# RunpeiDong/ACT

Measured on AMD Instinct MI355X. Metric: stage2_pretrain_point_clouds_per_sec, higher is better.
Workload: dtype f32

## Files before the change

act_amd/_abi.py:

```python
import ctypes

_vp, _i, _f, _sz = ctypes.c_void_p, ctypes.c_int, ctypes.c_float, ctypes.c_size_t
_u, _u64, _ll, _str = ctypes.c_uint, ctypes.c_uint64, ctypes.c_longlong, ctypes.c_char_p
_d = ctypes.c_double
_P = ctypes.POINTER


class GemmEpilogue(ctypes.Structure):
    _fields_ = [("alpha", _f), ("act", _i), ("accumulate", _i), ("rows_per_scale", _i), ("ldr", _i), ("ldaux", _i),
                ("res_row_div", _i), ("bias", _vp), ("rowscale", _vp), ("res", _vp), ("aux", _vp)]


class GemmTnProblem(ctypes.Structure):
    _fields_ = [("A", _vp), ("lda", _i), ("B", _vp), ("ldb", _i), ("C", _vp), ("ldc", _i), ("M", _i), ("N", _i), ("bias_out", _vp)]


class GemmFx(ctypes.Structure):
    _fields_ = ([(n, _vp) for n in ("a_scale", "a_shift", "b_scale", "b_shift", "tile_stats", "gmax", "garg")] + [("group", _i), ("store_c", _i)]
                + [(n, _vp) for n in ("sa_src", "sa_arg", "ep_src", "ep_arg", "row_groups")])


class BlockParams(ctypes.Structure):
    _fields_ = [(n, _vp) for n in ("norm1_w", "norm1_b", "qkv_w", "qkv_b", "proj_w", "proj_b", "norm2_w", "norm2_b",
                                   "fc1_w", "fc1_b", "fc2_w", "fc2_b")]
# ... 129 lines not shown
    "act_group_max_bwd_wgrad_workspace": (_sz, [_i, _i, _i, _i]),
    "act_group_max_bwd_wgrad_f32": [_vp, _vp, _i, _i, _i, _vp, _i, _i, _vp, _vp, _vp, _i, _vp, _sz, _vp],
    "act_group_sum_f32": [_vp, _i, _i, _i, _vp, _vp],
    "act_edge_gn_lrelu_max_f32": [_vp, _i, _i, _vp, _i, _i, _i, _i, _i, _vp, _vp, _f, _f, _vp, _vp, _i, _i, _vp],
    "act_edge_gn_lrelu_max_bwd_f32": [_vp, _i, _i, _vp, _i, _i, _i, _i, _i, _vp, _vp, _vp, _f, _vp, _i, _vp, _vp, _vp, _vp],
    "act_edge_bwd_lds": [_i],
    "act_gn_gumbel_argmax_gather_f32": [_vp, _i, _i, _i, _i, _vp, _vp, _f, _f, _vp, _u64, _vp, _f, _vp, _i, _vp, _vp, _vp, _vp, _vp],
    "act_gumbel_softmax_fwd_f32": [_vp, _i, _i, _vp, _u64, _f, _vp, _vp],
    "act_gumbel_softmax_bwd_f32": [_vp, _vp, _i, _i, _f, _vp, _vp],
    "act_kl_uniform_fwd_f32": [_vp, _i, _i, _i, _vp, _vp, _vp, _vp],
    "act_kl_uniform_bwd_f32": [_vp, _vp, _vp, _vp, _i, _i, _i, _vp, _vp],
    "act_split_bf16x2_f32": [_vp, _i, _i, _i, _vp, _vp, _vp],
    "act_sgemm_nt_bf16x3_supported": [_i, _i, _i],
    "act_sgemm_nt_bf16x3_f32": [_i, _i, _i, _vp, _vp, _vp, _vp, _vp, _i, _epi, _vp],
    "act_layernorm_fwd_planes_f32": [_vp, _vp, _vp, _vp, _vp, _vp, _vp, _vp, _vp, _vp, _i, _i, _f, _vp],
    "act_prompt_layernorm_fwd_planes_f32": [_vp, _vp, _i, _i, _i, _f, _u64, _vp, _vp, _vp, _f, _vp, _vp, _vp],
    "act_attention_fwd_prefix_planes_f32": [_vp, _i, _vp, _i, _vp, _vp, _vp, _vp, _i, _i, _i, _f, _vp],
    "act_sgemm_nt_bf16x3_planes_f32": [_i, _i, _i, _vp, _vp, _vp, _vp, _vp, _i, _vp, _vp, _epi, _vp],
    "act_split_f16x2_f32": [_vp, _i, _i, _i, _f, _vp, _vp, _vp, _vp],
    "act_sgemm_nt_f16x3_supported": [_i, _i, _i],
    "act_sgemm_nt_f16x3_planes_f32": [_i, _i, _i, _vp, _vp, _f, _vp, _vp, _vp, _vp, _i, _vp, _vp, _f, _epi, _vp],
    "act_sgemm_nt_f16x3_pick_tile": [_i, _i, _i, _i],
    "act_sgemm_nt_f16x3_planes_tile_f32": [_i, _i, _i, _vp, _vp, _f, _vp, _vp, _vp, _vp, _i, _vp, _vp, _f, _epi, _vp, _i],
    "act_layernorm_fwd_f16_planes_f32": [_vp, _vp, _vp, _vp, _vp, _vp, _vp, _vp, _f, _vp, _vp, _i, _i, _f, _vp],
    "act_attention_fwd_prefix_f16_planes_f32": [_vp, _i, _vp, _i, _vp, _vp, _vp, _f, _vp, _i, _i, _i, _f, _vp],
    "act_split_f16x2_affine_relu_f32": [_vp, _i, _i, _i, _vp, _vp, _f, _vp, _vp, _vp],
    "act_sgemm_nt_f16x3_gmax_supported": [_i, _i, _i, _i],
    "act_sgemm_nt_f16x3_gmax_pick_tile": [_i, _i, _i, _i],
    "act_sgemm_nt_f16x3_gmax_f32": [_i, _i, _i, _vp, _i, _vp, _vp, _vp, _vp, _f, _vp, _vp, _vp, _vp, _i, _vp, _i, _i, _vp],
    "act_gemm_tune_set": [_i] * 7,
    "act_gemm_tune_get": [_i] * 5 + [_P(_i), _P(_i)],
    "act_gemm_tune_clear": [],
    "act_gemm_tile_info": [_i] + [_P(_i)] * 4,
    "act_scale_rows_f32": [_vp, _vp, _i, _i, _i, _vp, _vp],
    "act_bn_eval_affine_f32": [_vp, _vp, _vp, _vp, _f, _i, _vp, _vp, _vp],
    "act_composite_collect_begin": [],
    "act_composite_collect_end": [_P(_i), _i],
    "act_composite_shutdown": [],
    "act_block_saved_floats": (_sz, [_dims]),
    "act_block_fwd_f32": [_dims, _blk, _vp, _vp, _vp, _vp, _i, _vp, _vp, _vp, _sz, _vp],
    "act_block_bwd_scratch_floats": (_sz, [_dims]),
    "act_block_bwd_f32": [_dims, _blk, _vp, _vp, _vp, _vp, _vp, _blk, _vp, _vp, _sz, _vp, _sz, _vp, _vp],
    "act_block_stack_saved_floats": (_sz, [_dims, _i, _i]),
    "act_block_stack_bwd_scratch_floats": (_sz, [_dims, _i]),
    "act_block_stack_fwd_f32": [_dims, _P(BlockStack), _vp, _vp, _i, _vp, _vp, _vp, _sz, _vp],
    "act_block_stack_bwd_f32": [_dims, _P(BlockStack), _vp, _vp, _vp, _vp, _vp, _vp, _vp, _vp, _sz, _vp, _sz, _vp, _vp],
# ... 108 lines not shown
```

act_amd/csrc/gemm_bf16x3.hip:

```cpp
#include "gemm_common.h"
#include "split_planes.h"
#include <stdlib.h>

typedef short bf16x8 __attribute__((ext_vector_type(8)));
typedef _Float16 f16x8 __attribute__((ext_vector_type(8)));
typedef unsigned u32x4v __attribute__((ext_vector_type(4)));

namespace {

__device__ __forceinline__ float4 x3_affine_relu4(const float4& a, const float4& sc, const float4& sh) {
    return make_float4(fmaxf(__builtin_fmaf(a.x, sc.x, sh.x), 0.f), fmaxf(__builtin_fmaf(a.y, sc.y, sh.y), 0.f),
                       fmaxf(__builtin_fmaf(a.z, sc.z, sh.z), 0.f), fmaxf(__builtin_fmaf(a.w, sc.w, sh.w), 0.f));
}
__device__ __forceinline__ float4 x3_scale4(const float4& a, float s) { return make_float4(a.x * s, a.y * s, a.z * s, a.w * s); }

template <bool F16, bool AFF = false>
__global__ __launch_bounds__(256) void split_planes_kernel(const float* __restrict__ x, int K4, int ldx, long long n4, float scale,
                                                           const float* __restrict__ row_scale, unsigned short* __restrict__ p1, unsigned short* __restrict__ p2,
                                                           const float* __restrict__ col_scale = nullptr, const float* __restrict__ col_shift = nullptr) {
    for (long long i = (long long)blockIdx.x * blockDim.x + threadIdx.x; i < n4; i += (long long)gridDim.x * blockDim.x) {
        const long long row = i / K4; const int c4 = (int)(i - row * K4);
        const float4 v = *reinterpret_cast<const float4*>(x + row * ldx + c4 * 4);
        if constexpr (AFF) {
            const float4 sc = x3_scale4(*reinterpret_cast<const float4*>(col_scale + c4 * 4), scale), sh = x3_scale4(*reinterpret_cast<const float4*>(col_shift + c4 * 4), scale);
// ... 21 lines not shown
__device__ __forceinline__ void x3_affine_split8(const u32x4v& a0, const u32x4v& a1, const float* sc, const float* sh, u32x4v& h1, u32x4v& h2) {
#pragma unroll
    for (int half = 0; half < 2; ++half) {
        const float4 c = *reinterpret_cast<const float4*>(sc + half * (LROW / 2)), s = *reinterpret_cast<const float4*>(sh + half * (LROW / 2));
        const float4 v = x3_affine_relu4(__builtin_bit_cast(float4, half ? a1 : a0), c, s);
        const float e[4] = {v.x, v.y, v.z, v.w};
        unsigned h[4], l[4];
#pragma unroll
        for (int j = 0; j < 4; ++j) split_f16x2(e[j], h[j], l[j]);
        h1[2 * half] = h[0] | (h[1] << 16); h1[2 * half + 1] = h[2] | (h[3] << 16);
        h2[2 * half] = l[0] | (l[1] << 16); h2[2 * half + 1] = l[2] | (l[3] << 16);
        __builtin_amdgcn_sched_barrier(0);
    }
}

template <bool F16>
__device__ __forceinline__ f32x4 x3_mfma(const bf16x8& b, const bf16x8& a, const f32x4& c) {
    if constexpr (F16) return __builtin_amdgcn_mfma_f32_16x16x32_f16(__builtin_bit_cast(f16x8, b), __builtin_bit_cast(f16x8, a), c, 0, 0, 0);
    else return __builtin_amdgcn_mfma_f32_16x16x32_bf16(b, a, c, 0, 0, 0);
}

constexpr int x3_wgs_per_cu(int waves) { return waves <= 4 ? 2 : 1; }

template <int BM, int BN, int WGM, int WGN, int ACT, bool PLANES, bool F16, bool A32 = false, bool GMAX = false>
__global__ __launch_bounds__(64 * WGM * WGN, x3_wgs_per_cu(WGM * WGN) * WGM * WGN / 4) void sgemm_nt_bf16x3_kernel(const X3Params p) {
    static_assert(F16 || !(A32 || GMAX), "the on-load split and the group max belong to the f16 form");
    static_assert(!GMAX || (BM / WGM == 64 && !PLANES), "a group of 32 or 64 rows lies inside one wave's 64-row block");
    constexpr int NT = 64 * WGM * WGN, RP = NT / 4;
    constexpr int WM = BM / WGM, WN = BN / WGN;
    constexpr int TM = WM / 16, TN = WN / 16;
    constexpr int PA = BM * LROW, PB = BN * LROW;
    constexpr int NA = (BM + RP - 1) / RP, NB = (BN + RP - 1) / RP;
    constexpr int STAGE = 2 * (PA + PB);
    static_assert(WM % 16 == 0 && WN % 16 == 0 && BM % 16 == 0 && BN % 16 == 0, "whole 16 x 16 blocks per wave, whole waves per staging row test");
    __shared__ __attribute__((aligned(16))) unsigned short L[2 * STAGE];
    const int tid = threadIdx.x, lane = tid & 63, wave = tid >> 6;
    const int wm = wave / WGN, wn = wave % WGN;
    const int tiles_n = p.N / BN, tiles_m = p.M / BM;
    int wg = blockIdx.x;
    {
        const int nwg = tiles_m * tiles_n, q = nwg >> 3, r = nwg & 7, xcd = wg & 7, loc = wg >> 3;
        wg = (xcd < r ? xcd * (q + 1) : r * (q + 1) + (xcd - r) * q) + loc;
    }
    constexpr int GM = 8;
    const int per_group = GM * tiles_n, group = wg / per_group, first_m = group * GM;
    const int gsz = min(tiles_m - first_m, GM), in_group = wg - group * per_group;
    const int tile_m = first_m + in_group % gsz, tile_n = in_group / gsz;
    const int m0 = tile_m * BM, n0 = tile_n * BN;
    const int K = p.K, ntiles = K / BK, last = ntiles - 1;

    constexpr int X = F16 ? 1 : 0;
    f32x4 acc[X + 1][TM][TN];
#pragma unroll
    for (int x = 0; x <= X; ++x)
// ... 25 lines not shown
                RA[s_][i_] = *reinterpret_cast<const u32x4v*>(gA[s_] + (X3_WHOLE(i_, BM) ? (long long)(RP * i_) * K : ta) + (T) * BK);  \
        _Pragma("unroll") for (int i_ = 0; i_ < NB; ++i_)                                                                              \
            RB[s_][i_] = *reinterpret_cast<const u32x4v*>(gB[s_] + (X3_WHOLE(i_, BN) ? (long long)(RP * i_) * K : tb) + (T) * BK);      \
    }
#define X3_STORE(RA, RB, STG, T)                                                                                                       \
    if constexpr (A32) {                                                                                                               \
        __builtin_amdgcn_sched_barrier(0);                                                                                             \
        _Pragma("unroll") for (int i_ = 0; i_ < NA; ++i_)                                                                              \
            if (X3_WHOLE(i_, BM) || srow + RP * i_ < BM) {                                                                             \
                u32x4v h1_, h2_;                                                                                                       \
                x3_affine_split8(RA[0][i_], RA[1][i_], Lf + sx_off + (T) * 8 * (LROW / 2), Lf + PA / 2 + sx_off + (T) * 8 * (LROW / 2), h1_, h2_); \
                *reinterpret_cast<u32x4v*>(&L[(STG) * STAGE + s_off + RP * i_ * LROW]) = h1_;                                          \
                *reinterpret_cast<u32x4v*>(&L[(STG) * STAGE + PA + s_off + RP * i_ * LROW]) = h2_;                                     \
            }                                                                                                                          \
    }                                                                                                                                  \
    _Pragma("unroll") for (int s_ = 0; s_ < 2; ++s_) {                                                                                 \
        _Pragma("unroll") for (int i_ = 0; i_ < NA; ++i_)                                                                              \
            if (!A32 && (X3_WHOLE(i_, BM) || srow + RP * i_ < BM))                                                                     \
                *reinterpret_cast<u32x4v*>(&L[(STG) * STAGE + s_ * PA + s_off + RP * i_ * LROW]) = RA[s_][i_];                         \
        _Pragma("unroll") for (int i_ = 0; i_ < NB; ++i_)                                                                              \
            if (X3_WHOLE(i_, BN) || srow + RP * i_ < BN)                                                                               \
                *reinterpret_cast<u32x4v*>(&L[(STG) * STAGE + 2 * PA + s_ * PB + s_off + RP * i_ * LROW]) = RB[s_][i_];                \
    }
#define X3_COMPUTE(STG)                                                                                                                \
    {                                                                                                                                  \
        const unsigned short* As_ = L + (STG) * STAGE; const unsigned short* Bs_ = As_ + 2 * PA;                                       \
        bf16x8 af[TM][2];                                                                                                              \
        _Pragma("unroll") for (int i_ = 0; i_ < TM; ++i_)                                                                              \
            _Pragma("unroll") for (int s_ = 0; s_ < 2; ++s_) af[i_][s_] = *reinterpret_cast<const bf16x8*>(&As_[s_ * PA + a_off + i_ * 16 * LROW]); \
        _Pragma("unroll") for (int j_ = 0; j_ < TN; ++j_) {                                                                            \
            bf16x8 bf[2];                                                                                                              \
            _Pragma("unroll") for (int s_ = 0; s_ < 2; ++s_) bf[s_] = *reinterpret_cast<const bf16x8*>(&Bs_[s_ * PB + b_off + j_ * 16 * LROW]); \
             \
             \
            _Pragma("unroll") for (int i_ = 0; i_ < TM; ++i_) acc[X][i_][j_] = x3_mfma<F16>(bf[0], af[i_][1], acc[X][i_][j_]);           \
            _Pragma("unroll") for (int i_ = 0; i_ < TM; ++i_) acc[X][i_][j_] = x3_mfma<F16>(bf[1], af[i_][0], acc[X][i_][j_]);           \
            _Pragma("unroll") for (int i_ = 0; i_ < TM; ++i_) acc[0][i_][j_] = x3_mfma<F16>(bf[0], af[i_][0], acc[0][i_][j_]);           \
        }                                                                                                                              \
    }
    X3_LOAD(ra0, rb0, 0)
    X3_LOAD(ra1, rb1, min(1, last))
    if constexpr (A32) {
        float* Lw = reinterpret_cast<float*>(L);
        for (int q = tid; q < K / 4; q += NT) {
            *reinterpret_cast<float4*>(&Lw[q * (LROW / 2) + 16]) = x3_scale4(*reinterpret_cast<const float4*>(p.a_sc + 4 * q), p.a_fold);
            *reinterpret_cast<float4*>(&Lw[PA / 2 + q * (LROW / 2) + 16]) = x3_scale4(*reinterpret_cast<const float4*>(p.a_sh + 4 * q), p.a_fold);
        }
        __syncthreads();
    }
    X3_STORE(ra0, rb0, 0, 0)
    __syncthreads();
    for (int t = 0; t < ntiles; t += 2) {
        X3_LOAD(ra0, rb0, min(t + 2, last))
        X3_COMPUTE(0)
        X3_STORE(ra1, rb1, 1, min(t + 1, last))
        __syncthreads();
        X3_LOAD(ra1, rb1, min(t + 3, last))
        X3_COMPUTE(1)
        X3_STORE(ra0, rb0, 0, min(t + 2, last))
        __syncthreads();
    }
#undef X3_WHOLE
#undef X3_LOAD
#undef X3_STORE
#undef X3_COMPUTE
    const bool vec = (((uintptr_t)p.C | (uintptr_t)p.epi.bias | (uintptr_t)p.epi.res | (uintptr_t)p.epi.aux) & 15) == 0 &&
                     ((p.ldc | (p.epi.res ? p.epi.ldr : 0) | (p.epi.aux ? p.epi.ldaux : 0)) & 3) == 0;
    auto value = [&](int i, int j, int row, int col) -> float4 {
        float4 v = make_float4(acc[0][i][j][0], acc[0][i][j][1], acc[0][i][j][2], acc[0][i][j][3]);
        if constexpr (F16) {
            const float4 bi = *reinterpret_cast<const float4*>(p.b_inv + col);
            constexpr float W = 1.0f / 2048.0f;
            v.x = __builtin_fmaf(acc[1][i][j][0], W, v.x) * bi.x * p.a_inv; v.y = __builtin_fmaf(acc[1][i][j][1], W, v.y) * bi.y * p.a_inv;
            v.z = __builtin_fmaf(acc[1][i][j][2], W, v.z) * bi.z * p.a_inv; v.w = __builtin_fmaf(acc[1][i][j][3], W, v.w) * bi.w * p.a_inv;
        }
        if (vec) v = epilogue_apply4_act<ACT>(p.epi, v, row, col);
        else {
            v.x = epilogue_apply<ACT>(p.epi, v.x, row, col); v.y = epilogue_apply<ACT>(p.epi, v.y, row, col + 1);
            v.z = epilogue_apply<ACT>(p.epi, v.z, row, col + 2); v.w = epilogue_apply<ACT>(p.epi, v.w, row, col + 3);
        }
        return v;
    };
    if constexpr (GMAX) {
        constexpr float NINF = -__builtin_huge_valf();
#pragma unroll
        for (int j = 0; j < TN; ++j) {
            const int col = n0 + wn * WN + j * 16 + g * 4;
            float4 m[2] = {make_float4(NINF, NINF, NINF, NINF), make_float4(NINF, NINF, NINF, NINF)};
// ... 15 lines not shown
                if (r == 0) {
                    float* cp = p.C + (size_t)((m0 + wm * WM + h * 32) / p.group) * p.ldc + col;
                    if (vec) *reinterpret_cast<float4*>(cp) = m[h]; else { cp[0] = m[h].x; cp[1] = m[h].y; cp[2] = m[h].z; cp[3] = m[h].w; }
                }
            }
        }
        return;
    }
#pragma unroll
    for (int i = 0; i < TM; ++i)
#pragma unroll
        for (int j = 0; j < TN; ++j) {
            const int row = m0 + wm * WM + i * 16 + r;
            const int col = n0 + wn * WN + j * 16 + g * 4;
            const float4 v = value(i, j, row, col);
            if (!PLANES || p.C) {
                float* cp = p.C + (size_t)row * p.ldc + col;
                if (vec) *reinterpret_cast<float4*>(cp) = v; else { cp[0] = v.x; cp[1] = v.y; cp[2] = v.z; cp[3] = v.w; }
            }
            if constexpr (PLANES) store_planes4<F16>(p.Oh, p.Ol, ((size_t)row * p.N + col) >> 2, v, p.o_scale);
        }
}

template <int BM, int BN, int WGM, int WGN, bool F16>
int launch_x3(const X3Params& p, hipStream_t s) {
    const dim3 grid((p.M / BM) * (p.N / BN)), block(64 * WGM * WGN);
    const bool planes = p.Oh != nullptr;
    switch (p.epi.act) {
        case ACT_EPI_NONE:
            if (planes) hipLaunchKernelGGL((sgemm_nt_bf16x3_kernel<BM, BN, WGM, WGN, ACT_EPI_NONE, true, F16>), grid, block, 0, s, p);
            else        hipLaunchKernelGGL((sgemm_nt_bf16x3_kernel<BM, BN, WGM, WGN, ACT_EPI_NONE, false, F16>), grid, block, 0, s, p);
            break;
        case ACT_EPI_GELU:
            if (planes) hipLaunchKernelGGL((sgemm_nt_bf16x3_kernel<BM, BN, WGM, WGN, ACT_EPI_GELU, true, F16>), grid, block, 0, s, p);
            else        hipLaunchKernelGGL((sgemm_nt_bf16x3_kernel<BM, BN, WGM, WGN, ACT_EPI_GELU, false, F16>), grid, block, 0, s, p);
            break;
        case ACT_EPI_MUL_GELU_GRAD:
            if (planes) hipLaunchKernelGGL((sgemm_nt_bf16x3_kernel<BM, BN, WGM, WGN, ACT_EPI_MUL_GELU_GRAD, true, F16>), grid, block, 0, s, p);
            else        hipLaunchKernelGGL((sgemm_nt_bf16x3_kernel<BM, BN, WGM, WGN, ACT_EPI_MUL_GELU_GRAD, false, F16>), grid, block, 0, s, p);
            break;
        default: return ACT_E_BADARG;
    }
    ACT_LAUNCH_CHECK();
    return 0;
}

template <int BM, int BN, int WGM, int WGN>
int launch_x3_gmax(const X3Params& p, bool a32, hipStream_t s) {
    const dim3 grid((p.M / BM) * (p.N / BN)), block(64 * WGM * WGN);
    if (a32) hipLaunchKernelGGL((sgemm_nt_bf16x3_kernel<BM, BN, WGM, WGN, ACT_EPI_NONE, false, true, true, true>), grid, block, 0, s, p);
    else     hipLaunchKernelGGL((sgemm_nt_bf16x3_kernel<BM, BN, WGM, WGN, ACT_EPI_NONE, false, true, false, true>), grid, block, 0, s, p);
    ACT_LAUNCH_CHECK();
    return 0;
}

template <bool F16>
int split_planes(const float* x, int R, int K, int ldx, float scale, const float* row_scale, uint16_t* p1, uint16_t* p2, act_stream_t stream) {
    if (!x || !p1 || !p2) return ACT_E_NULLPTR;
    if (R < 0 || K <= 0 || (K & 3) || ldx < K || (ldx & 3) || (F16 && !(scale > 0.f)) || (((uintptr_t)x | (uintptr_t)p1 | (uintptr_t)p2) & 15)) return ACT_E_BADARG;
    const long long n4 = (long long)R * K / 4; if (n4 == 0) return 0;
    hipStream_t s = (hipStream_t)stream;
    ActProfScope ps(KID_ELTWISE, s, 0.0, 8.0 * R * (double)K);
// ... 4 lines not shown

}

extern "C" int act_split_bf16x2_f32(const float* x, int R, int K, int ldx, uint16_t* hi, uint16_t* lo, act_stream_t stream) {
    return split_planes<false>(x, R, K, ldx, 0.f, nullptr, hi, lo, stream);
}
extern "C" int act_split_f16x2_f32(const float* x, int R, int K, int ldx, float scale, const float* row_scale, uint16_t* h1, uint16_t* h2,
                                   act_stream_t stream) {
    return split_planes<true>(x, R, K, ldx, scale, row_scale, h1, h2, stream);
}

extern "C" int act_sgemm_nt_bf16x3_supported(int M, int N, int K) { return M > 0 && N > 0 && K > 0 && M % 128 == 0 && N % 128 == 0 && K % 64 == 0; }
extern "C" int act_sgemm_nt_f16x3_supported(int M, int N, int K) { return act_sgemm_nt_bf16x3_supported(M, N, K); }

extern "C" int act_sgemm_nt_f16x3_pick_tile(int M, int N, int K, int cus) {
    if (!act_sgemm_nt_f16x3_supported(M, N, K) || cus <= 0) return 0;
    if (N % 384) return 128;
    const long long t128 = (long long)(M / 128) * (N / 128), t192 = (long long)(M / 128) * (N / 192);
    const long long tail = t128 % (2 * cus);
    const long long c128 = t128 / (2 * cus) * 4 + (tail == 0 ? 0 : tail <= cus ? 2 : 4), c192 = (t192 + cus - 1) / cus * 3;
    return 8 * c192 <= 7 * c128 ? 192 : 128;
}

namespace {
int x3_cu_count() {
    static const int n = [] {
        int dev = 0, v = 0;
        if (hipGetDevice(&dev) != hipSuccess || hipDeviceGetAttribute(&v, hipDeviceAttributeMultiprocessorCount, dev) != hipSuccess || v <= 0) v = 256;
        return v;
    }();
    return n;
}
bool x3_only_128() {
    static const bool v = [] { const char* e = getenv("ACT_X3_TILE"); return e && atoi(e) == 128; }();
    return v;
}
template <bool F16>
int multiply_planes(int M, int N, int K, const uint16_t* a1, const uint16_t* a2, float a_scale, const uint16_t* b1, const uint16_t* b2, const float* b_inv,
                    float* C, int ldc, uint16_t* o1, uint16_t* o2, float out_scale, const act_gemm_epilogue_t* epilogue, act_stream_t stream, int tile) {
    if (!a1 || !a2 || !b1 || !b2 || (F16 && !b_inv) || (!C && !o1) || ((o1 == nullptr) != (o2 == nullptr))) return ACT_E_NULLPTR;
    if (!act_sgemm_nt_bf16x3_supported(M, N, K) || (C && ldc < N) || (F16 && (!(a_scale > 0.f) || (o1 && !(out_scale > 0.f))))) return ACT_E_BADARG;
    if ((((uintptr_t)a1 | (uintptr_t)a2 | (uintptr_t)b1 | (uintptr_t)b2 | (uintptr_t)o1 | (uintptr_t)o2 | (uintptr_t)b_inv) & 15)) return ACT_E_BADARG;
    if (F16 && tile != 0 && tile != 128 && !(tile == 192 && N % 192 == 0)) return ACT_E_BADARG;
    if (F16 && tile == 0) tile = x3_only_128() ? 128 : act_sgemm_nt_f16x3_pick_tile(M, N, K, x3_cu_count());
    X3Params p{};
    p.Ah = a1; p.Al = a2; p.Bh = b1; p.Bl = b2; p.C = C; p.ldc = ldc; p.M = M; p.N = N; p.K = K; p.Oh = o1; p.Ol = o2;
    if (F16) { p.b_inv = b_inv; p.a_inv = 1.0f / a_scale; p.o_scale = out_scale; }
    if (epilogue) p.epi = *epilogue; else { p.epi = act_gemm_epilogue_t{}; p.epi.alpha = 1.0f; }
    if (p.epi.accumulate || (p.epi.act != ACT_EPI_NONE && p.epi.act != ACT_EPI_GELU && p.epi.act != ACT_EPI_MUL_GELU_GRAD)) return ACT_E_BADARG;
    hipStream_t s = (hipStream_t)stream;
    ActProfScope ps(KID_GEMM_BF16X3, s, 2.0 * M * (double)N * K, 4.0 * ((double)M * K + (double)N * K + (double)M * N));
    if constexpr (F16) return tile == 192 ? launch_x3<128, 192, 2, 4, true>(p, s) : launch_x3<128, 128, 2, 2, true>(p, s);
    else return launch_x3<128, 128, 2, 2, false>(p, s);
}
}

extern "C" int act_split_f16x2_affine_relu_f32(const float* x, int R, int K, int ldx, const float* col_scale, const float* col_shift, float scale, uint16_t* h1,
                                               uint16_t* h2, act_stream_t stream) {
    if (!x || !col_scale || !col_shift || !h1 || !h2) return ACT_E_NULLPTR;
    if (R < 0 || K <= 0 || (K & 3) || ldx < K || (ldx & 3) || !(scale > 0.f)) return ACT_E_BADARG;
    if (((uintptr_t)x | (uintptr_t)h1 | (uintptr_t)h2 | (uintptr_t)col_scale | (uintptr_t)col_shift) & 15) return ACT_E_BADARG;
    const long long n4 = (long long)R * K / 4; if (n4 == 0) return 0;
    hipStream_t s = (hipStream_t)stream;
    ActProfScope ps(KID_ELTWISE, s, 0.0, 8.0 * R * (double)K);
    long long g = (n4 + 255) / 256; if (g > 8192) g = 8192;
    hipLaunchKernelGGL((split_planes_kernel<true, true>), dim3((unsigned)g), dim3(256), 0, s, x, K / 4, ldx, n4, scale, nullptr, h1, h2, col_scale, col_shift);
    ACT_LAUNCH_CHECK(); return 0;
}
extern "C" int act_sgemm_nt_f16x3_gmax_supported(int M, int N, int K, int group) {
    return act_sgemm_nt_f16x3_supported(M, N, K) && K <= 512 && (group == 32 || group == 64);
}
extern "C" int act_sgemm_nt_f16x3_gmax_pick_tile(int M, int N, int K, int cus) { return act_sgemm_nt_f16x3_pick_tile(M, N, K, cus); }
extern "C" int act_sgemm_nt_f16x3_gmax_f32(int M, int N, int K, const float* A, int lda, const float* a_col_scale, const float* a_col_shift,
                                           const uint16_t* a_h1, const uint16_t* a_h2, float a_scale, const uint16_t* b_h1, const uint16_t* b_h2,
                                           const float* b_inv_scale, const float* bias, int group, float* out, int ldo, int tile, act_stream_t stream) {
    const bool a32 = A != nullptr;
// ... 4 lines not shown
    if (tile != 0 && tile != 128 && !(tile == 192 && N % 192 == 0)) return ACT_E_BADARG;
    if (tile == 0) tile = x3_only_128() ? 128 : act_sgemm_nt_f16x3_gmax_pick_tile(M, N, K, x3_cu_count());
    X3Params p{};
    p.A32 = A; p.lda = lda; p.a_sc = a_col_scale; p.a_sh = a_col_shift; p.a_fold = a_scale; p.Ah = a_h1; p.Al = a_h2; p.Bh = b_h1; p.Bl = b_h2;
    p.C = out; p.ldc = ldo; p.M = M; p.N = N; p.K = K; p.group = group; p.b_inv = b_inv_scale; p.a_inv = 1.0f / a_scale;
    p.epi = act_gemm_epilogue_t{}; p.epi.alpha = 1.0f; p.epi.bias = bias;
    hipStream_t s = (hipStream_t)stream;
    ActProfScope ps(KID_GEMM_BF16X3, s, 2.0 * M * (double)N * K, 4.0 * ((double)M * K + (double)N * K + (double)(M / group) * N));
    return tile == 192 ? launch_x3_gmax<128, 192, 2, 4>(p, a32, s) : launch_x3_gmax<128, 128, 2, 2>(p, a32, s);
}

extern "C" int act_sgemm_nt_bf16x3_f32(int M, int N, int K, const uint16_t* a_hi, const uint16_t* a_lo, const uint16_t* b_hi, const uint16_t* b_lo,
                                       float* C, int ldc, const act_gemm_epilogue_t* epilogue, act_stream_t stream) {
    return multiply_planes<false>(M, N, K, a_hi, a_lo, 0.f, b_hi, b_lo, nullptr, C, ldc, nullptr, nullptr, 0.f, epilogue, stream, 128);
}
extern "C" int act_sgemm_nt_bf16x3_planes_f32(int M, int N, int K, const uint16_t* a_hi, const uint16_t* a_lo, const uint16_t* b_hi, const uint16_t* b_lo,
                                              float* C, int ldc, uint16_t* out_hi, uint16_t* out_lo, const act_gemm_epilogue_t* epilogue,
                                              act_stream_t stream) {
    return multiply_planes<false>(M, N, K, a_hi, a_lo, 0.f, b_hi, b_lo, nullptr, C, ldc, out_hi, out_lo, 0.f, epilogue, stream, 128);
}
extern "C" int act_sgemm_nt_f16x3_planes_f32(int M, int N, int K, const uint16_t* a_h1, const uint16_t* a_h2, float a_scale, const uint16_t* b_h1,
                                             const uint16_t* b_h2, const float* b_inv_scale, float* C, int ldc, uint16_t* out_h1, uint16_t* out_h2,
                                             float out_scale, const act_gemm_epilogue_t* epilogue, act_stream_t stream) {
    return multiply_planes<true>(M, N, K, a_h1, a_h2, a_scale, b_h1, b_h2, b_inv_scale, C, ldc, out_h1, out_h2, out_scale, epilogue, stream, 0);
}
extern "C" int act_sgemm_nt_f16x3_planes_tile_f32(int M, int N, int K, const uint16_t* a_h1, const uint16_t* a_h2, float a_scale, const uint16_t* b_h1,
                                                  const uint16_t* b_h2, const float* b_inv_scale, float* C, int ldc, uint16_t* out_h1, uint16_t* out_h2,
                                                  float out_scale, const act_gemm_epilogue_t* epilogue, act_stream_t stream, int tile) {
    return multiply_planes<true>(M, N, K, a_h1, a_h2, a_scale, b_h1, b_h2, b_inv_scale, C, ldc, out_h1, out_h2, out_scale, epilogue, stream, tile);
}
```

act_amd/kernels.py:

```python
import ctypes
import os

import numpy as np

import torch

from . import _C
from ._abi import GemmEpilogue, GemmTnProblem

EPI_NONE, EPI_GELU, EPI_RELU, EPI_MUL_GELU_GRAD, EPI_MUL_RELU_MASK = 0, 1, 2, 3, 4

lib, ptr, stream, check = _C.lib, _C.ptr, _C.stream, _C.check

_WS = {}
_WS_BYTES = 160 << 20


def workspace(device, nbytes=_WS_BYTES, stream_handle=None):
    idx = device.index if device.index is not None else torch.cuda.current_device()
    key = (idx, _C.stream_handle(idx) if stream_handle is None else stream_handle)
    w = _WS.get(key)
    if w is None or w.numel() * 4 < nbytes:
        w = torch.empty(max(nbytes, _WS_BYTES) // 4, dtype=torch.float32, device=device)
        _WS[key] = w
# ... 165 lines not shown
    one = torch.ones(e.shape, dtype=torch.float32, device=w.device)
    return torch.ldexp(one, 15 - e), torch.ldexp(one, e - 15)


def split_f16x2(x, scale=1.0, row_scale=None, out=None):
    x = _f32rows(x, "x")
    R, Kd = x.shape
    if out is None:
        out = torch.empty(2, R, Kd, dtype=torch.float16, device=x.device)
    check(lib.act_split_f16x2_f32(_C.ptr_rows(x), R, Kd, x.stride(0), float(scale), ptr(_f32c(row_scale)) if row_scale is not None else None,
                                  ptr(out[0]), ptr(out[1]), stream()), "act_split_f16x2_f32")
    return out


def layernorm_f16_planes(x, gamma, beta, eps, scale, pos=None):
    x = _f32c(x)
    T, D = x.shape
    planes = torch.empty(2, T, D, dtype=torch.float16, device=x.device)
    check(lib.act_layernorm_fwd_f16_planes_f32(ptr(x), ptr(_f32c(pos)) if pos is not None else None, ptr(gamma), ptr(beta), None, None, ptr(planes[0]),
                                               ptr(planes[1]), float(scale), None, None, T, D, float(eps), stream()), "act_layernorm_fwd_f16_planes_f32")
    return planes


def gemm_nt_f16x3(a_planes, a_scale, b_planes, b_inv_scale, bias=None, act=EPI_NONE, res=None, out=None, planes_out=None, out_scale=1.0, tile=0):
    M, N, Kd, a1, a2, b1, b2, out, o1, o2, e = _x3_problem("gemm_nt_f16x3", torch.float16, a_planes, b_planes, bias, act, res, out, planes_out)
    b_inv_scale = _f32c(b_inv_scale)
    if b_inv_scale.numel() != N:
        raise _C.ActHipError("gemm_nt_f16x3: b_inv_scale must hold one value per row of b")
    check(lib.act_sgemm_nt_f16x3_planes_tile_f32(M, N, Kd, a1, a2, float(a_scale), b1, b2, ptr(b_inv_scale), ptr(out), out.stride(0), o1, o2, float(out_scale),
                                                 ctypes.byref(e), stream(), int(tile)), "act_sgemm_nt_f16x3_planes_tile_f32")
    return out


def split_f16x2_affine_relu(x, col_scale, col_shift, scale):
    x = _f32rows(x, "x")
    R, Kd = x.shape
    out = torch.empty(2, R, Kd, dtype=torch.float16, device=x.device)
    check(lib.act_split_f16x2_affine_relu_f32(_C.ptr_rows(x), R, Kd, x.stride(0), ptr(_f32c(col_scale)), ptr(_f32c(col_shift)), float(scale), ptr(out[0]),
                                              ptr(out[1]), stream()), "act_split_f16x2_affine_relu_f32")
    return out


def gemm_nt_f16x3_gmax(a, a_scale, b_planes, b_inv_scale, group, bias=None, col_scale=None, col_shift=None, tile=0):
    planes = a.dtype == torch.float16
    b_planes, b_inv_scale = b_planes.contiguous(), _f32c(b_inv_scale)
    N, Kd = b_planes.shape[1], b_planes.shape[2]
    if planes:
        a = a.contiguous()
        M = a.shape[1]
        args = (None, 0, None, None, ptr(a[0]), ptr(a[1]))
    else:
# ... 2241 lines not shown
```

include/act_hip.h:

```cpp
#ifndef ACT_HIP_H
#define ACT_HIP_H
#include <stdint.h>
#include <stddef.h>
#ifdef __cplusplus
extern "C" {
#endif

typedef void* act_stream_t;

#define ACT_E_BADARG   (-1)
#define ACT_E_NULLPTR  (-2)
#define ACT_E_UNSUPPORTED (-3)

int         act_version(void);
const char* act_arch(void);

int         act_prof_enable(int on);
int         act_prof_reset(void);
int         act_prof_num_kernels(void);
const char* act_prof_kernel_name(int id);
int         act_prof_read(int id, double* total_ms, long long* launches, double* flops, double* bytes);

size_t act_fps_scratch_floats(int B, int N);
int act_fps_f32(const float* xyz, int B, int N, int G, int32_t* idx_out, float* centers_out,
// ... 184 lines not shown
int act_sgemm_nt_bf16x3_supported(int M, int N, int K);
int act_sgemm_nt_bf16x3_f32(int M, int N, int K, const uint16_t* a_hi, const uint16_t* a_lo, const uint16_t* b_hi, const uint16_t* b_lo,
                            float* C, int ldc, const act_gemm_epilogue_t* epilogue, act_stream_t stream);
int act_layernorm_fwd_planes_f32(const float* x, const float* pos, const float* gamma, const float* beta, float* xin_out, float* y,
                                 uint16_t* y_hi, uint16_t* y_lo, float* mean , float* rstd , int T, int D, float eps,
                                 act_stream_t stream);
int act_prompt_layernorm_fwd_planes_f32(const float* tok, const float* ppos, int B, int P, int D, float drop_p, uint64_t seed,
                                        const uint64_t* seed_dev, const float* gamma, const float* beta, float eps, uint16_t* y_hi, uint16_t* y_lo,
                                        act_stream_t stream);
int act_attention_fwd_prefix_planes_f32(const float* kv0, int S0, const float* qkv1, int Sq, float* out, uint16_t* out_hi, uint16_t* out_lo, float* lse,
                                        int B, int H, int head_dim, float scale, act_stream_t stream);
int act_sgemm_nt_bf16x3_planes_f32(int M, int N, int K, const uint16_t* a_hi, const uint16_t* a_lo, const uint16_t* b_hi, const uint16_t* b_lo,
                                   float* C, int ldc, uint16_t* out_hi, uint16_t* out_lo, const act_gemm_epilogue_t* epilogue, act_stream_t stream);

int act_split_f16x2_f32(const float* x, int R, int K, int ldx, float scale, const float* row_scale, uint16_t* h1, uint16_t* h2, act_stream_t stream);
int act_sgemm_nt_f16x3_supported(int M, int N, int K);
int act_sgemm_nt_f16x3_planes_f32(int M, int N, int K, const uint16_t* a_h1, const uint16_t* a_h2, float a_scale, const uint16_t* b_h1,
                                  const uint16_t* b_h2, const float* b_inv_scale, float* C, int ldc, uint16_t* out_h1, uint16_t* out_h2, float out_scale,
                                  const act_gemm_epilogue_t* epilogue, act_stream_t stream);
int act_sgemm_nt_f16x3_pick_tile(int M, int N, int K, int cus);
int act_sgemm_nt_f16x3_planes_tile_f32(int M, int N, int K, const uint16_t* a_h1, const uint16_t* a_h2, float a_scale, const uint16_t* b_h1,
                                       const uint16_t* b_h2, const float* b_inv_scale, float* C, int ldc, uint16_t* out_h1, uint16_t* out_h2,
                                       float out_scale, const act_gemm_epilogue_t* epilogue, act_stream_t stream, int tile);
int act_layernorm_fwd_f16_planes_f32(const float* x, const float* pos, const float* gamma, const float* beta, float* xin_out, float* y,
                                     uint16_t* y_h1, uint16_t* y_h2, float plane_scale, float* mean , float* rstd , int T, int D,
                                     float eps, act_stream_t stream);
int act_attention_fwd_prefix_f16_planes_f32(const float* kv0, int S0, const float* qkv1, int Sq, float* out, uint16_t* out_h1, uint16_t* out_h2,
                                            float plane_scale, float* lse, int B, int H, int head_dim, float scale, act_stream_t stream);
int act_split_f16x2_affine_relu_f32(const float* x, int R, int K, int ldx, const float* col_scale, const float* col_shift, float scale, uint16_t* h1,
                                    uint16_t* h2, act_stream_t stream);
int act_sgemm_nt_f16x3_gmax_supported(int M, int N, int K, int group);
int act_sgemm_nt_f16x3_gmax_pick_tile(int M, int N, int K, int cus);
int act_sgemm_nt_f16x3_gmax_f32(int M, int N, int K, const float* A, int lda, const float* a_col_scale, const float* a_col_shift, const uint16_t* a_h1,
                                const uint16_t* a_h2, float a_scale, const uint16_t* b_h1, const uint16_t* b_h2, const float* b_inv_scale,
                                const float* bias, int group, float* out, int ldo, int tile, act_stream_t stream);

int act_gemm_tune_set(int a_kmajor, int b_kmajor, int M, int N, int K, int tile, int splits);
int act_gemm_tune_get(int a_kmajor, int b_kmajor, int M, int N, int K, int* tile, int* splits);
int act_gemm_tune_clear(void);
#define ACT_GEMM_LAYOUT_TN 1
#define ACT_GEMM_LAYOUT_TT 2
#define ACT_GEMM_LAYOUT_NN 4
#define ACT_GEMM_LAYOUT_NT 8
#define ACT_GEMM_NEED_ANY           0
#define ACT_GEMM_NEED_FULL_OR_MTAIL 1
#define ACT_GEMM_NEED_FULL          2
// ... 301 lines not shown
```

Before: 6995.

## Add direct global-to-LDS DMA form for f16x3 plane GEMM with swizzled 64-wide K tiles

Adds a K64 variant of the split-f16 GEMM kernel that uses global_load_lds to copy 64-wide K slices of the four planes straight into a swizzled LDS image. This removes the register round trip and LDS store pass of the old load/store pipeline, and it runs with 8 waves and an XOR chunk swizzle to avoid bank conflicts. A heuristic picks this form and its tile by default for 192-wide tiles or small grids. The cost is a full vmcnt(0) wait plus a barrier at every stage, and the new path requires K to be a multiple of 64.

```diff
diff --git a/act_amd/_abi.py b/act_amd/_abi.py
--- a/act_amd/_abi.py
+++ b/act_amd/_abi.py
@@ -175,6 +175,10 @@
     "act_sgemm_nt_f16x3_planes_f32": [_i, _i, _i, _vp, _vp, _f, _vp, _vp, _vp, _vp, _i, _vp, _vp, _f, _epi, _vp],
     "act_sgemm_nt_f16x3_pick_tile": [_i, _i, _i, _i],
     "act_sgemm_nt_f16x3_planes_tile_f32": [_i, _i, _i, _vp, _vp, _f, _vp, _vp, _vp, _vp, _i, _vp, _vp, _f, _epi, _vp, _i],
+    "act_sgemm_nt_f16x3_pick_form": [_i, _i, _i, _i],
+    "act_sgemm_nt_f16x3_k64_pick_tile": [_i, _i, _i, _i],
+    "act_sgemm_nt_f16x3_planes_form_f32": [_i, _i, _i, _vp, _vp, _f, _vp, _vp, _vp, _vp, _i, _vp, _vp, _f, _epi, _vp, _i, _i],
+    "act_x3_k64_image_chunk": [_i, _i],
     "act_layernorm_fwd_f16_planes_f32": [_vp, _vp, _vp, _vp, _vp, _vp, _vp, _vp, _f, _vp, _vp, _i, _i, _f, _vp],
     "act_attention_fwd_prefix_f16_planes_f32": [_vp, _i, _vp, _i, _vp, _vp, _vp, _f, _vp, _i, _i, _i, _f, _vp],
     "act_split_f16x2_affine_relu_f32": [_vp, _i, _i, _i, _vp, _vp, _f, _vp, _vp, _vp],
diff --git a/act_amd/csrc/gemm_bf16x3.hip b/act_amd/csrc/gemm_bf16x3.hip
--- a/act_amd/csrc/gemm_bf16x3.hip
+++ b/act_amd/csrc/gemm_bf16x3.hip
@@ -1,5 +1,6 @@
 #include "gemm_common.h"
 #include "split_planes.h"
+#include "x3_lds_image.h"
 #include <stdlib.h>
 
 typedef short bf16x8 __attribute__((ext_vector_type(8)));
@@ -67,14 +68,16 @@
 
 constexpr int x3_wgs_per_cu(int waves) { return waves <= 4 ? 2 : 1; }
 
-template <int BM, int BN, int WGM, int WGN, int ACT, bool PLANES, bool F16, bool A32 = false, bool GMAX = false>
+template <int BM, int BN, int WGM, int WGN, int ACT, bool PLANES, bool F16, bool A32 = false, bool GMAX = false, bool K64 = false>
 __global__ __launch_bounds__(64 * WGM * WGN, x3_wgs_per_cu(WGM * WGN) * WGM * WGN / 4) void sgemm_nt_bf16x3_kernel(const X3Params p) {
     static_assert(F16 || !(A32 || GMAX), "the on-load split and the group max belong to the f16 form");
     static_assert(!GMAX || (BM / WGM == 64 && !PLANES), "a group of 32 or 64 rows lies inside one wave's 64-row block");
+    static_assert(!K64 || (F16 && !A32 && !GMAX && WGM * WGN == 8 && BM % 64 == 0 && BN % 64 == 0), "the DMA form: f16 planes in, 8 waves, whole 64-row bands per plane");
     constexpr int NT = 64 * WGM * WGN, RP = NT / 4;
     constexpr int WM = BM / WGM, WN = BN / WGN;
     constexpr int TM = WM / 16, TN = WN / 16;
-    constexpr int PA = BM * LROW, PB = BN * LROW;
+    constexpr int PITCH = K64 ? 64 : LROW;
+    constexpr int PA = BM * PITCH, PB = BN * PITCH;
     constexpr int NA = (BM + RP - 1) / RP, NB = (BN + RP - 1) / RP;
     constexpr int STAGE = 2 * (PA + PB);
     static_assert(WM % 16 == 0 && WN % 16 == 0 && BM % 16 == 0 && BN % 16 == 0, "whole 16 x 16 blocks per wave, whole waves per staging row test");
@@ -146,15 +149,16 @@
             if (X3_WHOLE(i_, BN) || srow + RP * i_ < BN)                                                                               \
                 *reinterpret_cast<u32x4v*>(&L[(STG) * STAGE + 2 * PA + s_ * PB + s_off + RP * i_ * LROW]) = RB[s_][i_];                \
     }
-#define X3_COMPUTE(STG)                                                                                                                \
+#define X3_COMPUTE(STG) X3_COMPUTE_AT(STG, a_off, b_off)
+#define X3_COMPUTE_AT(STG, AO, BO)                                                                                                     \
     {                                                                                                                                  \
         const unsigned short* As_ = L + (STG) * STAGE; const unsigned short* Bs_ = As_ + 2 * PA;                                       \
         bf16x8 af[TM][2];                                                                                                              \
         _Pragma("unroll") for (int i_ = 0; i_ < TM; ++i_)                                                                              \
-            _Pragma("unroll") for (int s_ = 0; s_ < 2; ++s_) af[i_][s_] = *reinterpret_cast<const bf16x8*>(&As_[s_ * PA + a_off + i_ * 16 * LROW]); \
+            _Pragma("unroll") for (int s_ = 0; s_ < 2; ++s_) af[i_][s_] = *reinterpret_cast<const bf16x8*>(&As_[s_ * PA + (AO) + i_ * 16 * PITCH]); \
         _Pragma("unroll") for (int j_ = 0; j_ < TN; ++j_) {                                                                            \
             bf16x8 bf[2];                                                                                                              \
-            _Pragma("unroll") for (int s_ = 0; s_ < 2; ++s_) bf[s_] = *reinterpret_cast<const bf16x8*>(&Bs_[s_ * PB + b_off + j_ * 16 * LROW]); \
+            _Pragma("unroll") for (int s_ = 0; s_ < 2; ++s_) bf[s_] = *reinterpret_cast<const bf16x8*>(&Bs_[s_ * PB + (BO) + j_ * 16 * PITCH]); \
              \
              \
             _Pragma("unroll") for (int i_ = 0; i_ < TM; ++i_) acc[X][i_][j_] = x3_mfma<F16>(bf[0], af[i_][1], acc[X][i_][j_]);           \
@@ -162,32 +166,78 @@
             _Pragma("unroll") for (int i_ = 0; i_ < TM; ++i_) acc[0][i_][j_] = x3_mfma<F16>(bf[0], af[i_][0], acc[0][i_][j_]);           \
         }                                                                                                                              \
     }
-    X3_LOAD(ra0, rb0, 0)
-    X3_LOAD(ra1, rb1, min(1, last))
-    if constexpr (A32) {
-        float* Lw = reinterpret_cast<float*>(L);
-        for (int q = tid; q < K / 4; q += NT) {
-            *reinterpret_cast<float4*>(&Lw[q * (LROW / 2) + 16]) = x3_scale4(*reinterpret_cast<const float4*>(p.a_sc + 4 * q), p.a_fold);
-            *reinterpret_cast<float4*>(&Lw[PA / 2 + q * (LROW / 2) + 16]) = x3_scale4(*reinterpret_cast<const float4*>(p.a_sh + 4 * q), p.a_fold);
-        }
+    if constexpr (K64) {
+        constexpr int PPA = BM / 8, PPB = BN / 8, NPW = (2 * PPA + 2 * PPB) / 8;
+        const int wv = __builtin_amdgcn_readfirstlane(wave);
+        const int prow = 8 * wv + (lane >> 3), pch = x3_k64_image_chunk(prow, lane & 7);
+        const unsigned voff = (unsigned)(prow * K + pch * 8) * 2u;
+        const size_t oa = (size_t)m0 * K, ob = (size_t)n0 * K;
+        const unsigned short* src[4] = {p.Ah + oa, p.Al + oa, p.Bh + ob, p.Bl + ob};
+        static_assert(WM % 16 == 0 && WN % 16 == 0, "the map's row term is that of r alone");
+        const int a64[2] = {(wm * WM + r) * PITCH + x3_k64_image_chunk(r, g) * 8, (wm * WM + r) * PITCH + x3_k64_image_chunk(r, 4 + g) * 8};
+        const int b64[2] = {(wn * WN + r) * PITCH + x3_k64_image_chunk(r, g) * 8, (wn * WN + r) * PITCH + x3_k64_image_chunk(r, 4 + g) * 8};
+        typedef const __attribute__((address_space(1))) void* gptr_t;
+        typedef __attribute__((address_space(3))) void* lptr_t;
+#define X3_DMA(STG, T)                                                                                                                 \
+        const unsigned vo_##STG = voff + (unsigned)(T) * 128u;                                                                         \
+        _Pragma("unroll") for (int i_ = 0; i_ < NPW; ++i_) {                                                                           \
+            const int pc_ = 8 * i_;                                                                      \
+            const int pl_ = pc_ < PPA ? 0 : pc_ < 2 * PPA ? 1 : pc_ < 2 * PPA + PPB ? 2 : 3;                                           \
+            const int band_ = (pc_ - (pl_ == 0 ? 0 : pl_ == 1 ? PPA : pl_ == 2 ? 2 * PPA : 2 * PPA + PPB)) / 8;                        \
+            __builtin_amdgcn_global_load_lds((gptr_t)((const char*)(src[pl_] + (size_t)band_ * 64 * K) + vo_##STG),                    \
+                                             (lptr_t)(L + (STG) * STAGE + (pc_ + wv) * 512), 16, 0, 0);                                \
+        }
+#define X3_DMA_LANDED()                                                                                                                \
+        asm volatile("s_waitcnt vmcnt(0)" ::: "memory"); asm volatile("s_waitcnt lgkmcnt(0)" ::: "memory");                            \
+        __builtin_amdgcn_s_barrier(); asm volatile("" ::: "memory");
+        const int last64 = K / 64 - 1;
+        { X3_DMA(0, 0) }
+        X3_DMA_LANDED()
+        for (int t = 1; t <= last64; t += 2) {
+            { X3_DMA(1, t) }
+            X3_COMPUTE_AT(0, a64[0], b64[0])
+            X3_COMPUTE_AT(0, a64[1], b64[1])
+            X3_DMA_LANDED()
+            { X3_DMA(0, min(t + 1, last64)) }
+            X3_COMPUTE_AT(1, a64[0], b64[0])
+            X3_COMPUTE_AT(1, a64[1], b64[1])
+            X3_DMA_LANDED()
+        }
+        if (!(last64 & 1)) {
+            X3_COMPUTE_AT(0, a64[0], b64[0])
+            X3_COMPUTE_AT(0, a64[1], b64[1])
+        }
+#undef X3_DMA
+#undef X3_DMA_LANDED
+    } else {
+        X3_LOAD(ra0, rb0, 0)
+        X3_LOAD(ra1, rb1, min(1, last))
+        if constexpr (A32) {
+            float* Lw = reinterpret_cast<float*>(L);
+            for (int q = tid; q < K / 4; q += NT) {
+                *reinterpret_cast<float4*>(&Lw[q * (LROW / 2) + 16]) = x3_scale4(*reinterpret_cast<const float4*>(p.a_sc + 4 * q), p.a_fold);
+                *reinterpret_cast<float4*>(&Lw[PA / 2 + q * (LROW / 2) + 16]) = x3_scale4(*reinterpret_cast<const float4*>(p.a_sh + 4 * q), p.a_fold);
+            }
+            __syncthreads();
+        }
+        X3_STORE(ra0, rb0, 0, 0)
         __syncthreads();
-    }
-    X3_STORE(ra0, rb0, 0, 0)
-    __syncthreads();
-    for (int t = 0; t < ntiles; t += 2) {
-        X3_LOAD(ra0, rb0, min(t + 2, last))
-        X3_COMPUTE(0)
-        X3_STORE(ra1, rb1, 1, min(t + 1, last))
-        __syncthreads();
-        X3_LOAD(ra1, rb1, min(t + 3, last))
-        X3_COMPUTE(1)
-        X3_STORE(ra0, rb0, 0, min(t + 2, last))
-        __syncthreads();
+        for (int t = 0; t < ntiles; t += 2) {
+            X3_LOAD(ra0, rb0, min(t + 2, last))
+            X3_COMPUTE(0)
+            X3_STORE(ra1, rb1, 1, min(t + 1, last))
+            __syncthreads();
+            X3_LOAD(ra1, rb1, min(t + 3, last))
+            X3_COMPUTE(1)
+            X3_STORE(ra0, rb0, 0, min(t + 2, last))
+            __syncthreads();
+        }
     }
 #undef X3_WHOLE
 #undef X3_LOAD
 #undef X3_STORE
 #undef X3_COMPUTE
+#undef X3_COMPUTE_AT
     const bool vec = (((uintptr_t)p.C | (uintptr_t)p.epi.bias | (uintptr_t)p.epi.res | (uintptr_t)p.epi.aux) & 15) == 0 &&
                      ((p.ldc | (p.epi.res ? p.epi.ldr : 0) | (p.epi.aux ? p.epi.ldaux : 0)) & 3) == 0;
     auto value = [&](int i, int j, int row, int col) -> float4 {
@@ -249,22 +299,22 @@
         }
 }
 
-template <int BM, int BN, int WGM, int WGN, bool F16>
+template <int BM, int BN, int WGM, int WGN, bool F16, bool K64 = false>
 int launch_x3(const X3Params& p, hipStream_t s) {
     const dim3 grid((p.M / BM) * (p.N / BN)), block(64 * WGM * WGN);
     const bool planes = p.Oh != nullptr;
     switch (p.epi.act) {
         case ACT_EPI_NONE:
-            if (planes) hipLaunchKernelGGL((sgemm_nt_bf16x3_kernel<BM, BN, WGM, WGN, ACT_EPI_NONE, true, F16>), grid, block, 0, s, p);
-            else        hipLaunchKernelGGL((sgemm_nt_bf16x3_kernel<BM, BN, WGM, WGN, ACT_EPI_NONE, false, F16>), grid, block, 0, s, p);
+            if (planes) hipLaunchKernelGGL((sgemm_nt_bf16x3_kernel<BM, BN, WGM, WGN, ACT_EPI_NONE, true, F16, false, false, K64>), grid, block, 0, s, p);
+            else        hipLaunchKernelGGL((sgemm_nt_bf16x3_kernel<BM, BN, WGM, WGN, ACT_EPI_NONE, false, F16, false, false, K64>), grid, block, 0, s, p);
             break;
         case ACT_EPI_GELU:
-            if (planes) hipLaunchKernelGGL((sgemm_nt_bf16x3_kernel<BM, BN, WGM, WGN, ACT_EPI_GELU, true, F16>), grid, block, 0, s, p);
-            else        hipLaunchKernelGGL((sgemm_nt_bf16x3_kernel<BM, BN, WGM, WGN, ACT_EPI_GELU, false, F16>), grid, block, 0, s, p);
+            if (planes) hipLaunchKernelGGL((sgemm_nt_bf16x3_kernel<BM, BN, WGM, WGN, ACT_EPI_GELU, true, F16, false, false, K64>), grid, block, 0, s, p);
+            else        hipLaunchKernelGGL((sgemm_nt_bf16x3_kernel<BM, BN, WGM, WGN, ACT_EPI_GELU, false, F16, false, false, K64>), grid, block, 0, s, p);
             break;
         case ACT_EPI_MUL_GELU_GRAD:
-            if (planes) hipLaunchKernelGGL((sgemm_nt_bf16x3_kernel<BM, BN, WGM, WGN, ACT_EPI_MUL_GELU_GRAD, true, F16>), grid, block, 0, s, p);
-            else        hipLaunchKernelGGL((sgemm_nt_bf16x3_kernel<BM, BN, WGM, WGN, ACT_EPI_MUL_GELU_GRAD, false, F16>), grid, block, 0, s, p);
+            if (planes) hipLaunchKernelGGL((sgemm_nt_bf16x3_kernel<BM, BN, WGM, WGN, ACT_EPI_MUL_GELU_GRAD, true, F16, false, false, K64>), grid, block, 0, s, p);
+            else        hipLaunchKernelGGL((sgemm_nt_bf16x3_kernel<BM, BN, WGM, WGN, ACT_EPI_MUL_GELU_GRAD, false, F16, false, false, K64>), grid, block, 0, s, p);
             break;
         default: return ACT_E_BADARG;
     }
@@ -315,6 +365,13 @@
     return 8 * c192 <= 7 * c128 ? 192 : 128;
 }
 
+extern "C" int act_sgemm_nt_f16x3_k64_pick_tile(int M, int N, int K, int cus) {
+    if (!act_sgemm_nt_f16x3_supported(M, N, K) || cus <= 0) return 0;
+    if (N % 384) return 128;
+    const long long t128 = (long long)(M / 128) * (N / 128), t192 = (long long)(M / 128) * (N / 192);
+    return (t192 + cus - 1) / cus * 3 <= (t128 + cus - 1) / cus * 2 ? 192 : 128;
+}
+
 namespace {
 int x3_cu_count() {
     static const int n = [] {
@@ -328,14 +385,29 @@
     static const bool v = [] { const char* e = getenv("ACT_X3_TILE"); return e && atoi(e) == 128; }();
     return v;
 }
+bool x3_form0_only() {
+    static const bool v = [] { const char* e = getenv("ACT_X3_FORM"); return e && atoi(e) == 0; }();
+    return v;
+}
+int x3_pick_form(int M, int N, int K, int cus, int tile) {
+    if (!act_sgemm_nt_f16x3_supported(M, N, K) || cus <= 0 || (tile != 128 && tile != 192)) return 0;
+    return tile == 192 || (long long)(M / 128) * (N / 128) <= 4LL * cus;
+}
+constexpr int X3_FORM_RULE = -1;
 template <bool F16>
 int multiply_planes(int M, int N, int K, const uint16_t* a1, const uint16_t* a2, float a_scale, const uint16_t* b1, const uint16_t* b2, const float* b_inv,
-                    float* C, int ldc, uint16_t* o1, uint16_t* o2, float out_scale, const act_gemm_epilogue_t* epilogue, act_stream_t stream, int tile) {
+                    float* C, int ldc, uint16_t* o1, uint16_t* o2, float out_scale, const act_gemm_epilogue_t* epilogue, act_stream_t stream, int tile,
+                    int form = 0) {
     if (!a1 || !a2 || !b1 || !b2 || (F16 && !b_inv) || (!C && !o1) || ((o1 == nullptr) != (o2 == nullptr))) return ACT_E_NULLPTR;
     if (!act_sgemm_nt_bf16x3_supported(M, N, K) || (C && ldc < N) || (F16 && (!(a_scale > 0.f) || (o1 && !(out_scale > 0.f))))) return ACT_E_BADARG;
     if ((((uintptr_t)a1 | (uintptr_t)a2 | (uintptr_t)b1 | (uintptr_t)b2 | (uintptr_t)o1 | (uintptr_t)o2 | (uintptr_t)b_inv) & 15)) return ACT_E_BADARG;
     if (F16 && tile != 0 && tile != 128 && !(tile == 192 && N % 192 == 0)) return ACT_E_BADARG;
-    if (F16 && tile == 0) tile = x3_only_128() ? 128 : act_sgemm_nt_f16x3_pick_tile(M, N, K, x3_cu_count());
+    if (form != X3_FORM_RULE && form != 0 && !(F16 && form == 1)) return ACT_E_BADARG;
+    if (F16 && tile == 0) {
+        const int cus = x3_cu_count(), t1 = x3_only_128() ? 128 : act_sgemm_nt_f16x3_k64_pick_tile(M, N, K, cus);
+        if (form == X3_FORM_RULE) form = x3_form0_only() ? 0 : x3_pick_form(M, N, K, cus, t1);
+        tile = form == 1 ? t1 : x3_only_128() ? 128 : act_sgemm_nt_f16x3_pick_tile(M, N, K, cus);
+    } else if (form == X3_FORM_RULE) form = 0;
     X3Params p{};
     p.Ah = a1; p.Al = a2; p.Bh = b1; p.Bl = b2; p.C = C; p.ldc = ldc; p.M = M; p.N = N; p.K = K; p.Oh = o1; p.Ol = o2;
     if (F16) { p.b_inv = b_inv; p.a_inv = 1.0f / a_scale; p.o_scale = out_scale; }
@@ -343,8 +415,10 @@
     if (p.epi.accumulate || (p.epi.act != ACT_EPI_NONE && p.epi.act != ACT_EPI_GELU && p.epi.act != ACT_EPI_MUL_GELU_GRAD)) return ACT_E_BADARG;
     hipStream_t s = (hipStream_t)stream;
     ActProfScope ps(KID_GEMM_BF16X3, s, 2.0 * M * (double)N * K, 4.0 * ((double)M * K + (double)N * K + (double)M * N));
-    if constexpr (F16) return tile == 192 ? launch_x3<128, 192, 2, 4, true>(p, s) : launch_x3<128, 128, 2, 2, true>(p, s);
-    else return launch_x3<128, 128, 2, 2, false>(p, s);
+    if constexpr (F16) {
+        if (form == 1) return tile == 192 ? launch_x3<128, 192, 2, 4, true, true>(p, s) : launch_x3<128, 128, 2, 4, true, true>(p, s);
+        return tile == 192 ? launch_x3<128, 192, 2, 4, true>(p, s) : launch_x3<128, 128, 2, 2, true>(p, s);
+    } else return launch_x3<128, 128, 2, 2, false>(p, s);
 }
 }
 
@@ -395,10 +469,21 @@
 extern "C" int act_sgemm_nt_f16x3_planes_f32(int M, int N, int K, const uint16_t* a_h1, const uint16_t* a_h2, float a_scale, const uint16_t* b_h1,
                                              const uint16_t* b_h2, const float* b_inv_scale, float* C, int ldc, uint16_t* out_h1, uint16_t* out_h2,
                                              float out_scale, const act_gemm_epilogue_t* epilogue, act_stream_t stream) {
-    return multiply_planes<true>(M, N, K, a_h1, a_h2, a_scale, b_h1, b_h2, b_inv_scale, C, ldc, out_h1, out_h2, out_scale, epilogue, stream, 0);
+    return multiply_planes<true>(M, N, K, a_h1, a_h2, a_scale, b_h1, b_h2, b_inv_scale, C, ldc, out_h1, out_h2, out_scale, epilogue, stream, 0, X3_FORM_RULE);
 }
 extern "C" int act_sgemm_nt_f16x3_planes_tile_f32(int M, int N, int K, const uint16_t* a_h1, const uint16_t* a_h2, float a_scale, const uint16_t* b_h1,
                                                   const uint16_t* b_h2, const float* b_inv_scale, float* C, int ldc, uint16_t* out_h1, uint16_t* out_h2,
                                                   float out_scale, const act_gemm_epilogue_t* epilogue, act_stream_t stream, int tile) {
-    return multiply_planes<true>(M, N, K, a_h1, a_h2, a_scale, b_h1, b_h2, b_inv_scale, C, ldc, out_h1, out_h2, out_scale, epilogue, stream, tile);
-}
+    return multiply_planes<true>(M, N, K, a_h1, a_h2, a_scale, b_h1, b_h2, b_inv_scale, C, ldc, out_h1, out_h2, out_scale, epilogue, stream, tile,
+                                 X3_FORM_RULE);
+}
+extern "C" int act_sgemm_nt_f16x3_pick_form(int M, int N, int K, int cus) {
+    return x3_pick_form(M, N, K, cus, act_sgemm_nt_f16x3_k64_pick_tile(M, N, K, cus));
+}
+extern "C" int act_sgemm_nt_f16x3_planes_form_f32(int M, int N, int K, const uint16_t* a_h1, const uint16_t* a_h2, float a_scale, const uint16_t* b_h1,
+                                                  const uint16_t* b_h2, const float* b_inv_scale, float* C, int ldc, uint16_t* out_h1, uint16_t* out_h2,
+                                                  float out_scale, const act_gemm_epilogue_t* epilogue, act_stream_t stream, int tile, int form) {
+    if (form != 0 && form != 1) return ACT_E_BADARG;
+    return multiply_planes<true>(M, N, K, a_h1, a_h2, a_scale, b_h1, b_h2, b_inv_scale, C, ldc, out_h1, out_h2, out_scale, epilogue, stream, tile, form);
+}
+extern "C" int act_x3_k64_image_chunk(int row, int chunk) { return row < 0 || chunk < 0 || chunk > 7 ? -1 : x3_k64_image_chunk(row, chunk); }
diff --git a/act_amd/csrc/x3_lds_image.h b/act_amd/csrc/x3_lds_image.h
--- /dev/null
+++ b/act_amd/csrc/x3_lds_image.h
@@ -0,0 +1,9 @@
+#pragma once
+
+#if defined(__HIPCC__) || defined(__CUDACC__)
+#define X3_IMAGE_FN __host__ __device__ constexpr
+#else
+#define X3_IMAGE_FN constexpr
+#endif
+
+X3_IMAGE_FN int x3_k64_image_chunk(int row, int chunk) { return chunk ^ ((row >> 1) & 7); }
diff --git a/act_amd/kernels.py b/act_amd/kernels.py
--- a/act_amd/kernels.py
+++ b/act_amd/kernels.py
@@ -211,11 +211,15 @@
     return planes
 
 
-def gemm_nt_f16x3(a_planes, a_scale, b_planes, b_inv_scale, bias=None, act=EPI_NONE, res=None, out=None, planes_out=None, out_scale=1.0, tile=0):
+def gemm_nt_f16x3(a_planes, a_scale, b_planes, b_inv_scale, bias=None, act=EPI_NONE, res=None, out=None, planes_out=None, out_scale=1.0, tile=0, form=None):
     M, N, Kd, a1, a2, b1, b2, out, o1, o2, e = _x3_problem("gemm_nt_f16x3", torch.float16, a_planes, b_planes, bias, act, res, out, planes_out)
     b_inv_scale = _f32c(b_inv_scale)
     if b_inv_scale.numel() != N:
         raise _C.ActHipError("gemm_nt_f16x3: b_inv_scale must hold one value per row of b")
+    if form is not None:
+        check(lib.act_sgemm_nt_f16x3_planes_form_f32(M, N, Kd, a1, a2, float(a_scale), b1, b2, ptr(b_inv_scale), ptr(out), out.stride(0), o1, o2,
+                                                     float(out_scale), ctypes.byref(e), stream(), int(tile), int(form)), "act_sgemm_nt_f16x3_planes_form_f32")
+        return out
     check(lib.act_sgemm_nt_f16x3_planes_tile_f32(M, N, Kd, a1, a2, float(a_scale), b1, b2, ptr(b_inv_scale), ptr(out), out.stride(0), o1, o2, float(out_scale),
                                                  ctypes.byref(e), stream(), int(tile)), "act_sgemm_nt_f16x3_planes_tile_f32")
     return out
diff --git a/include/act_hip.h b/include/act_hip.h
--- a/include/act_hip.h
+++ b/include/act_hip.h
@@ -230,6 +230,12 @@
 int act_sgemm_nt_f16x3_planes_tile_f32(int M, int N, int K, const uint16_t* a_h1, const uint16_t* a_h2, float a_scale, const uint16_t* b_h1,
                                        const uint16_t* b_h2, const float* b_inv_scale, float* C, int ldc, uint16_t* out_h1, uint16_t* out_h2,
                                        float out_scale, const act_gemm_epilogue_t* epilogue, act_stream_t stream, int tile);
+int act_sgemm_nt_f16x3_pick_form(int M, int N, int K, int cus);
+int act_sgemm_nt_f16x3_k64_pick_tile(int M, int N, int K, int cus);
+int act_sgemm_nt_f16x3_planes_form_f32(int M, int N, int K, const uint16_t* a_h1, const uint16_t* a_h2, float a_scale, const uint16_t* b_h1,
+                                       const uint16_t* b_h2, const float* b_inv_scale, float* C, int ldc, uint16_t* out_h1, uint16_t* out_h2,
+                                       float out_scale, const act_gemm_epilogue_t* epilogue, act_stream_t stream, int tile, int form);
+int act_x3_k64_image_chunk(int row, int chunk);
 int act_layernorm_fwd_f16_planes_f32(const float* x, const float* pos, const float* gamma, const float* beta, float* xin_out, float* y,
                                      uint16_t* y_h1, uint16_t* y_h2, float plane_scale, float* mean , float* rstd , int T, int D,
                                      float eps, act_stream_t stream);
```

New measurement: 7016 (median of 6 runs). About the same (+0.3%).
